# KikeM/romtime

Measured on AMD Instinct MI355X. Metric: snapshot-DoF/s for POD build, higher is better.
Workload: dtype f64

## Files before the change

### include/romtime_hip.h

```cpp
#ifndef ROMTIME_HIP_H
#define ROMTIME_HIP_H

#include <stdint.h>

#ifdef __cplusplus
extern "C" {
#endif

typedef struct rt_ctx rt_ctx;

#define RT_OK 0
#define RT_ERR_ARG (-1)
#define RT_ERR_HIP (-2)
#define RT_ERR_UNSUPPORTED (-3)
#define RT_WARN_ZERO_NORM 1
#define RT_WARN_SINGULAR 2

#define RT_ROW_MAJOR 0
#define RT_COL_MAJOR 1

int rt_version(void);
int rt_ctx_create(rt_ctx** out, int device);
void rt_ctx_destroy(rt_ctx* ctx);
int rt_ctx_set_stream(rt_ctx* ctx, void* hip_stream);
// ... 108 lines not shown
  const double* C_nl;
  const double* S_nl;
} rt_hsweep_desc;
int rt_hrom_bdf_sweep(rt_ctx* ctx, const rt_hsweep_desc* desc, double* uN_out);
int rt_last_sweep_stats(rt_ctx* ctx, int64_t* stats4);

int rt_trajectory_errors(rt_ctx* ctx, const double* B, int64_t ldb, const double* A, int64_t lda, int64_t stride_a,
                         const double* U, int64_t ldu, int u_layout, int64_t stride_u, int64_t N, int64_t k, int64_t nt,
                         int64_t n_traj, double* err, double* ref);

#define RT_P1_MASS 0
#define RT_P1_STIFFNESS 1
#define RT_P1_CONVECTION 2
#define RT_P1_TRILINEAR 3
#define RT_P1_LOAD 4
#define RT_P1_LOAD_P2 5
int rt_p1_local_assembly(rt_ctx* ctx, int kind, int64_t nx, const int64_t* rows, const int64_t* cols, int64_t m,
                         int64_t n_states, const double* h, const double* coef, int state_mode, const double* state,
                         double* out);

int rt_sym_eig_values(rt_ctx* ctx, const double* G, int64_t n, double* lam, int* status);
int rt_sym_eig_values_part(rt_ctx* ctx, const double* G, int64_t n, int64_t first, int64_t count, double* lam,
                           int* status);
int rt_sym_eig_vectors(rt_ctx* ctx, int64_t n, int64_t k, const double* lam, double* W);

int rt_host_jacobi_eigh(double* A, int64_t n, double* W, double* lam, int max_sweeps, int* sweeps_done);

int rt_bench_mfma_f64(rt_ctx* ctx, int iters, double* tflops);
int rt_bench_copy(rt_ctx* ctx, void* dst, const void* src, int64_t bytes, int reps, double* gbps);

#ifdef __cplusplus
}
#endif
#endif
```

### romtime_amd/_lib.py

```python
from __future__ import annotations

import ctypes as C
import os
import threading
import weakref

_HERE = os.path.dirname(os.path.abspath(__file__))
LIB_PATH = os.path.join(_HERE, "lib", "libromtime_hip.so")

ROW_MAJOR, COL_MAJOR = 0, 1
RT_OK = 0
WARN_ZERO_NORM, WARN_SINGULAR = 1, 2

_p = C.c_void_p
_i64 = C.c_int64
_int = C.c_int

SOLVER_DIRECT, SOLVER_GMRES = 0, 1


class GmresOpts(C.Structure):

    _fields_ = [("rtol", C.c_double), ("atol", C.c_double), ("restart", _i64), ("maxiter", _i64)]

# ... 21 lines not shown
    "rt_pod_enqueue": (_int, [_p, _p, _i64, _i64, _i64, _int, _i64, _int, _p, _p, _p, _p, _p, _p, _p]),
    "rt_pod_orth": (_int, [_p, _p, _i64, _i64, _i64, _int, _i64, C.c_double, _int, _p, _i64, C.POINTER(_i64), _p, _p,
                           C.POINTER(_int)]),
    "rt_gemm_tn": (_int, [_p, _p, _i64, _int, _p, _i64, _int, _i64, _i64, _i64, _p, _i64]),
    "rt_gemm_nn": (_int, [_p, _p, _i64, _int, _p, _i64, _i64, _i64, _i64, _p, _i64, _int]),
    "rt_rank_update": (_int, [_p, _p, _i64, _p, _p, _i64, _p, _i64, _i64, _i64, _i64, C.c_double, _p, _i64]),
    "rt_gemm_nn_axpby": (_int, [_p, _p, _i64, _int, _p, _i64, _i64, _i64, _i64, C.c_double, C.c_double, _p, _i64, _int]),
    "rt_transpose": (_int, [_p, _p, _i64, _i64, _i64, _p, _i64]),
    "rt_deim_greedy": (_int, [_p, _p, _i64, _i64, _i64, _int, _p, _p, _p]),
    "rt_csr_spmm": (_int, [_p, _p, _p, _p, _i64, _p, _i64, _i64, _p, _i64]),
    "rt_project_csr": (_int, [_p, _p, _p, _p, _i64, _p, _i64, _i64, _p]),
    "rt_project_csr_batched": (_int, [_p, _p, _p, _p, _i64, _int, _i64, _i64, _p, _i64, _i64, _p]),
    "rt_dense_solve_batched": (_int, [_p, _p, _p, _i64, _i64, _p]),
    "rt_dense_solve_multi": (_int, [_p, _p, _i64, _p, _p, _i64, _p]),
    "rt_tracked_solve_batched": (_int, [_p, _p, _p, _p, _i64, _i64, _int, _p]),
    "rt_gmres_batched": (_int, [_p, _p, _p, _p, _i64, _i64, C.POINTER(GmresOpts), _p, _p]),
    "rt_ctx_set_reduced_solver": (_int, [_p, _int, C.POINTER(GmresOpts)]),
    "rt_rom_bdf_sweep": (_int, [_p, _p, _p]),
    "rt_hrom_bdf_sweep": (_int, [_p, _p, _p]),
    "rt_trajectory_errors": (_int, [_p, _p, _i64, _p, _i64, _i64, _p, _i64, _int, _i64, _i64, _i64, _i64, _i64, _p, _p]),
    "rt_p1_local_assembly": (_int, [_p, _int, _i64, _p, _p, _i64, _i64, _p, _p, _int, _p, _p]),
    "rt_sym_eig_values": (_int, [_p, _p, _i64, _p, _p]),
    "rt_sym_eig_values_part": (_int, [_p, _p, _i64, _i64, _i64, _p, _p]),
    "rt_sym_eig_vectors": (_int, [_p, _i64, _i64, _p, _p]),
    "rt_host_jacobi_eigh": (_int, [_p, _i64, _p, _p, _int, C.POINTER(_int)]),
    "rt_bench_mfma_f64": (_int, [_p, _int, C.POINTER(C.c_double)]),
    "rt_bench_copy": (_int, [_p, _p, _p, _i64, _int, C.POINTER(C.c_double)]),
}



class SweepDesc(C.Structure):

    _fields_ = [("N", _i64), ("nnz", _i64), ("r", _i64), ("n_mu", _i64), ("nt", _i64), ("dt", C.c_double),
                ("bdf2", _int), ("indptr", _p), ("indices", _p), ("V", _p), ("mass_values", _p), ("n_terms", _i64),
                ("term_values", _p), ("term_coef", _p), ("tril_values", _p), ("n_rhs", _i64), ("rhs_terms", _p),
                ("rhs_coef", _p)]


class HSweepDesc(C.Structure):

    _fields_ = [("r", _i64), ("n_mu", _i64), ("nt", _i64), ("dt", C.c_double), ("bdf2", _int), ("m_mass", _i64),
                ("m_lin", _i64), ("m_nl", _i64), ("m_rhs", _i64), ("Z", _p), ("Zf", _p), ("F_mass", _p), ("F_lin", _p),
                ("F_rhs", _p), ("W", _p), ("C_nl", _p), ("S_nl", _p)]


# ... 165 lines not shown
```

### romtime_amd/csrc/api.hip

```cpp
#include "common.h"

#include <chrono>
#include <new>

typedef double d4 __attribute__((ext_vector_type(4)));

namespace {

int grow(rt_ctx* ctx, void** buf, size_t* have, size_t bytes, void** out) {
  if (bytes > *have) {
    RT_HIP_CHECK(ctx, hipStreamSynchronize(ctx->stream));
    if (*buf) RT_HIP_CHECK(ctx, hipFree(*buf));
    *buf = nullptr;
    *have = 0;
    const size_t want = (bytes + ((size_t)1 << 20) - 1) & ~(((size_t)1 << 20) - 1);
    RT_HIP_CHECK(ctx, hipMalloc(buf, want));
    *have = want;
  }
  *out = *buf;
  return RT_OK;
}

__global__ void gram_scale_kernel(double* __restrict__ G, int n, double* __restrict__ colnorm, int normalize,
                                  int* status_flag) {
// ... 111 lines not shown
__global__ __launch_bounds__(256) void copy_kernel(double4* __restrict__ dst, const double4* __restrict__ src, long n4) {
  const long stride = (long)gridDim.x * blockDim.x;
  for (long i = (long)blockIdx.x * blockDim.x + threadIdx.x; i < n4; i += stride) dst[i] = src[i];
}

}

int rt_scratch(rt_ctx* ctx, size_t bytes, void** out) { return grow(ctx, &ctx->scratch, &ctx->scratch_bytes, bytes, out); }
int rt_scratch2(rt_ctx* ctx, size_t bytes, void** out) {
  ++ctx->scratch2_gen;
  return grow(ctx, &ctx->scratch2, &ctx->scratch2_bytes, bytes, out);
}

int rt_func_lds(rt_ctx* ctx, const void* fn, int bytes) {
  for (const void* f : ctx->lds_done)
    if (f == fn) return RT_OK;
  RT_HIP_CHECK(ctx, hipFuncSetAttribute(fn, hipFuncAttributeMaxDynamicSharedMemorySize, bytes));
  ctx->lds_done.push_back(fn);
  return RT_OK;
}

extern "C" {

int rt_version(void) { return 340; }

int rt_ctx_create(rt_ctx** out, int device) {
  if (!out) return RT_ERR_ARG;
  *out = nullptr;
  int count = 0;
  if (hipGetDeviceCount(&count) != hipSuccess || device < 0 || device >= count) return RT_ERR_HIP;
  if (hipSetDevice(device) != hipSuccess) return RT_ERR_HIP;
  rt_ctx* ctx = new (std::nothrow) rt_ctx();
  if (!ctx) return RT_ERR_HIP;
  ctx->device = device;
  hipDeviceProp_t prop;
  if (hipGetDeviceProperties(&prop, device) == hipSuccess) ctx->num_cus = ctx->device_cus = prop.multiProcessorCount;
  if (hipMalloc(reinterpret_cast<void**>(&ctx->dev_counters), sizeof(long) * RT_N_COUNTERS) != hipSuccess ||
      hipMemset(ctx->dev_counters, 0, sizeof(long) * RT_N_COUNTERS) != hipSuccess) {
    delete ctx;
    return RT_ERR_HIP;
  }
  *out = ctx;
  return RT_OK;
}

void rt_ctx_destroy(rt_ctx* ctx) {
  if (!ctx) return;
// ... 44 lines not shown
int rt_ctx_synchronize(rt_ctx* ctx) {
  if (!ctx) return RT_ERR_ARG;
  RT_HIP_CHECK(ctx, hipStreamSynchronize(ctx->stream));
  return RT_OK;
}

const char* rt_last_error(rt_ctx* ctx) { return ctx ? ctx->err.c_str() : "null ctx"; }

int rt_last_launch_info(rt_ctx* ctx, int64_t* info3) {
  if (!ctx || !info3) return RT_ERR_ARG;
  info3[0] = ctx->last_grid;
  info3[1] = ctx->last_splits;
  info3[2] = ctx->last_tile;
  return RT_OK;
}

int rt_ctx_set_option(rt_ctx* ctx, const char* name, int value) {
  if (!ctx || !name) return RT_ERR_ARG;
  const std::string key(name);
  if (key == "eig_one_xcd") {
    ctx->eig_one_xcd = value != 0;
    return RT_OK;
  }
  if (key == "eig_xcd") {
    if (value < 0 || value > 7) {
      ctx->err = "rt_ctx_set_option: eig_xcd must be 0 .. 7";
      return RT_ERR_ARG;
    }
    ctx->eig_xcd = value;
    return RT_OK;
  }
  if (key == "gram_pace") {
    ctx->gram_pace_on = value != 0;
    return RT_OK;
  }
  if (key == "sweep_graph") {
    ctx->sweep_graph = value != 0;
    return RT_OK;
  }
  if (key == "cu_limit") {
    if (value < 0 || value > ctx->device_cus || (value % 8) != 0) {
      ctx->err = "rt_ctx_set_option: cu_limit must be a multiple of 8 between 0 and the device's CU count";
      return RT_ERR_ARG;
    }
    ctx->num_cus = value ? value : ctx->device_cus;
    return RT_OK;
  }
  ctx->err = "rt_ctx_set_option: unknown option " + key;
  return RT_ERR_ARG;
}

int rt_ctx_get_counter(rt_ctx* ctx, const char* name, int64_t* value) {
  if (!ctx || !name || !value) return RT_ERR_ARG;
  const std::string key(name);
  static const struct { const char* name; int slot; } table[] = {
      {"eig_timeouts", RT_CNT_EIG_TIMEOUT}, {"eig_general_form", RT_CNT_EIG_GENERAL_FORM},
      {"eig_one_xcd", RT_CNT_EIG_ONE_XCD}, {"gram_off_xcd", RT_CNT_GRAM_OFF_XCD}, {"sweep_newton_iterations", RT_CNT_NS_ITER},
      {"sweep_restarts", RT_CNT_NS_RESTART}, {"sweep_lu_fallbacks", RT_CNT_LU_FALLBACK}, {"sweep_solves", RT_CNT_SOLVES},
      {"sweep_gmres_iterations", RT_CNT_GMRES_ITER}, {"sweep_gmres_unconverged", RT_CNT_GMRES_UNCONVERGED}};
  for (const auto& t : table)
    if (key == t.name) {
      long host = 0;
      RT_HIP_CHECK(ctx, hipMemcpyAsync(&host, ctx->dev_counters + t.slot, sizeof(long), hipMemcpyDeviceToHost, ctx->stream));
      RT_HIP_CHECK(ctx, hipStreamSynchronize(ctx->stream));
      *value = host;
      return RT_OK;
    }
  ctx->err = "rt_ctx_get_counter: unknown counter " + key;
  return RT_ERR_ARG;
}

int rt_last_sweep_stats(rt_ctx* ctx, int64_t* stats4) {
  if (!ctx || !stats4) return RT_ERR_ARG;
  long host[4];
  RT_HIP_CHECK(ctx, hipMemcpyAsync(host, ctx->dev_counters + RT_CNT_NS_ITER, sizeof(host), hipMemcpyDeviceToHost, ctx->stream));
  RT_HIP_CHECK(ctx, hipStreamSynchronize(ctx->stream));
  for (int i = 0; i < 4; ++i) stats4[i] = host[i];
  return RT_OK;
}

int rt_ctx_set_profile(rt_ctx* ctx, int on) {
  if (!ctx) return RT_ERR_ARG;
// ... 175 lines not shown
```

### romtime_amd/csrc/common.h

```cpp
#pragma once
#include <hip/hip_runtime.h>
#include <stdint.h>
#include <string>
#include <vector>

#include "../../include/romtime_hip.h"

constexpr int RT_N_COUNTERS = 10;

struct rt_ctx {
  int device = 0;
  hipStream_t stream = nullptr;
  void* scratch = nullptr;
  size_t scratch_bytes = 0;
  void* scratch2 = nullptr;
  size_t scratch2_bytes = 0;
  int num_cus = 256;
  int device_cus = 256;
  std::string err;
  int64_t last_grid = 0, last_splits = 0, last_tile = 0;
  bool profile = false;
  hipEvent_t ev0 = nullptr, ev1 = nullptr;
  bool ev_valid = false;
  hipEvent_t gev0 = nullptr, gev1 = nullptr;
  bool gev_valid = false;
  bool sweep_graph = false;
  bool eig_one_xcd = true;
  int eig_xcd = 0;
  struct {
    const double *d = nullptr, *e = nullptr, *V = nullptr, *tau = nullptr;
    int64_t n = 0;
    void* base = nullptr;
    uint64_t gen = 0;
  } eig;
  uint64_t scratch2_gen = 0;
  std::vector<const void*> lds_done;
  long* dev_counters = nullptr;
  unsigned long long* gram_pace = nullptr;
  bool gram_pace_on = true;
  int reduced_solver = RT_SOLVER_DIRECT;
  rt_gmres_opts gmres_opts{1e-5, 0.0, 20, 1};
};

enum {
  RT_CNT_EIG_TIMEOUT = 0,
  RT_CNT_EIG_GENERAL_FORM = 1,
  RT_CNT_EIG_ONE_XCD = 2,
  RT_CNT_GRAM_OFF_XCD = 3,
  RT_CNT_NS_ITER = 4,
  RT_CNT_NS_RESTART = 5,
  RT_CNT_LU_FALLBACK = 6,
  RT_CNT_SOLVES = 7,
  RT_CNT_GMRES_ITER = 8,
  RT_CNT_GMRES_UNCONVERGED = 9
};

#define RT_TRY(expr)                 \
  do {                               \
    const int _rc = (expr);          \
    if (_rc != RT_OK) return _rc;    \
  } while (0)

int rt_func_lds(rt_ctx* ctx, const void* fn, int bytes);

#define RT_HIP_CHECK(ctx, expr)                                                              \
  do {                                                                                       \
    hipError_t _e = (expr);                                                                  \
    if (_e != hipSuccess) {                                                                  \
      (ctx)->err = std::string(#expr) + ": " + hipGetErrorString(_e);                        \
      return RT_ERR_HIP;                                                                     \
    }                                                                                        \
  } while (0)

#define RT_ARG_CHECK(ctx, cond)                                                              \
  do {                                                                                       \
    if (!(cond)) {                                                                           \
      (ctx)->err = std::string("bad argument: ") + #cond;                                    \
// ... 40 lines not shown
```

### romtime_amd/csrc/symeig.hip

```cpp
#include "common.h"
#include "wave_ops.h"

namespace {

constexpr int TW_SMALL = 32;
constexpr int SLOT0 = 160;
constexpr int TW_LARGE = 128;
constexpr int LPR = 64;
constexpr int TT = 1024;
static_assert(LPR == 64, "row reductions use the whole-wave DPP sum");
constexpr int NMAX = 1024;
constexpr int VEC_ITERS = 2;

struct TriParams {
  const double* G;
  double* V;
  double* P;
  double* tau;
  double* d;
  double* e;
  int* flags;
  int n;
  int tw;
  int local;
// ... 310 lines not shown
  double q = d[0] - x;
  if (fabs(q) < pivmin) q = -pivmin;
  int c = (q < 0.0);
  for (int i = 1; i < n; ++i) {
    q = fma(-e2[i - 1], fast_rcp(q), d[i] - x);
    if (fabs(q) < pivmin) q = -pivmin;
    c += (q < 0.0);
  }
  return c;
}

__global__ void symeig_init_kernel(int* flags, double* tau, int n) {
  for (int i = threadIdx.x; i < SLOT0 + TW_LARGE; i += blockDim.x) flags[i] = 0;
  for (int i = threadIdx.x; i < n; i += blockDim.x) tau[i] = 0.0;
}

constexpr int BIS_NS = 2;
template <int NM>
__global__ __launch_bounds__(256) void symeig_bisect_kernel(const double* __restrict__ d, const double* __restrict__ e,
                                                            int n, int first, int count, double* __restrict__ lam,
                                                            const int* flags, int* status, long* counters) {
  if (blockIdx.x == 0 && threadIdx.x == 0) {
    if (status) *status = flags[3];
    if (flags[3]) atomicAdd(reinterpret_cast<unsigned long long*>(&counters[RT_CNT_EIG_TIMEOUT]), 1ull);
  }
  __shared__ double sd[NM], se2[NM];
  __shared__ int s_first[2][4];
  const int tid = threadIdx.x, lane = tid & 63, wid = tid >> 6, half = wid & 1;
  double glo = 1e300, ghi = -1e300, emax = 0.0;
  for (int i = lane; i < n; i += 64) {
    const double di = d[i], ei = (i + 1 < n) ? e[i] : 0.0, el = (i > 0) ? fabs(e[i - 1]) : 0.0;
    sd[i] = di;
    se2[i] = ei * ei;
    glo = fmin(glo, di - el - fabs(ei));
    ghi = fmax(ghi, di + el + fabs(ei));
    emax = fmax(emax, ei * ei);
  }
  glo = rtw::wave_min(glo);
  ghi = rtw::wave_max(ghi);
  emax = rtw::wave_max(emax);
  __syncthreads();
  const double tn = fmax(fabs(glo), fabs(ghi));
  double lo = glo - 2.2e-16 * tn * n - 1e-300, hi = ghi + 2.2e-16 * tn * n + 1e-300;
  const double pivmin = 2.2250738585072014e-308 * fmax(1.0, emax);
  const int j = first + min(2 * (int)blockIdx.x + (wid >> 1), count - 1);
  const int want = n - j;
  constexpr int NSH = 128 * BIS_NS;
// ... 11 lines not shown
      q0 = fma(-ei, fast_rcp(q0), di - x0);
      q1 = fma(-ei, fast_rcp(q1), di - x1);
      if (fabs(q0) < pivmin) q0 = -pivmin;
      if (fabs(q1) < pivmin) q1 = -pivmin;
      c0 += (q0 < 0.0); c1 += (q1 < 0.0);
    }
    int first = NSH;
    if (c1 >= want) first = s0 + 1;
    if (c0 >= want) first = s0;
    first = rtw::wave_min_i32(first);
    if (lane == 0) s_first[pass & 1][wid] = first;
    __syncthreads();
    first = min(s_first[pass & 1][wid & 2], s_first[pass & 1][(wid & 2) + 1]);
    if (first == NSH) {
      lo = lo + h * NSH;
    } else {
      hi = lo + h * (first + 1);
      lo = lo + h * first;
    }
  }
  if (lane == 0 && half == 0) lam[j] = 0.5 * (lo + hi);
}

struct VecParams {
  const double* d;
  const double* e;
  const double* lam;
  const double* V;
  const double* tau;
  const double* C;
  double* W;
  int n, k;
};

constexpr int RBK = 4;

template <int NM>
__global__ __launch_bounds__(64) void symeig_wy_kernel(const double* __restrict__ V, int n, double* __restrict__ C) {
  constexpr int PER = NM / 64;
  const int b = blockIdx.x, lane = threadIdx.x, k0 = n - 3 - RBK * b;
  double v[RBK][PER];
#pragma unroll
  for (int u = 0; u < RBK; ++u)
#pragma unroll
    for (int q = 0; q < PER; ++q) {
      const int k = k0 - u, j = lane + 64 * q;
// ... 126 lines not shown
      a[u] = dot;
    }
#pragma unroll
    for (int u = 0; u < RBK; ++u) a[u] = rtw::wave_sum(a[u]);
    const double s0 = tk[0] * a[0];
    const double s1 = tk[1] * (a[1] - cc[0] * s0);
    const double s2 = tk[2] * (a[2] - cc[1] * s0 - cc[2] * s1);
    const double s3 = tk[3] * (a[3] - cc[3] * s0 - cc[4] * s1 - cc[5] * s2);
#pragma unroll
    for (int q = 0; q < PER; ++q)
      zr[q] = fma(-s3, vc[3][q], fma(-s2, vc[2][q], fma(-s1, vc[1][q], fma(-s0, vc[0][q], zr[q]))));
#pragma unroll
    for (int u = 0; u < RBK; ++u)
#pragma unroll
      for (int q = 0; q < PER; ++q) vc[u][q] = vn[u][q];
  }
#pragma unroll
  for (int q = 0; q < PER; ++q) {
    const int j = lane + 64 * q;
    if (j < n) z[j] = zr[q];
  }
  __syncthreads();
  for (int i = lane; i < n; i += 64) p.W[(size_t)i * p.k + t] = z[i];
}

}

extern "C" int rt_sym_eig_values(rt_ctx* ctx, const double* G, int64_t n, double* lam, int* status) {
  return rt_sym_eig_values_part(ctx, G, n, 0, n, lam, status);
}

extern "C" int rt_sym_eig_values_part(rt_ctx* ctx, const double* G, int64_t n, int64_t first, int64_t count, double* lam,
                                      int* status) {
  if (!ctx) return RT_ERR_ARG;
  RT_ARG_CHECK(ctx, G && lam && n >= 3 && first >= 0 && count >= 1 && first + count <= n);
  if (n > NMAX) {
    ctx->err = "rt_sym_eig_values: n > 1024 not supported (the matrix must stay resident in the LDS of <= 128 CUs)";
    return RT_ERR_UNSUPPORTED;
  }
  const bool large = n > 512;
  const bool small_team = !large && ctx->num_cus < TW_SMALL && ctx->num_cus >= TW_SMALL / 2;
  int tw = large ? TW_LARGE : (small_team ? TW_SMALL / 2 : TW_SMALL);
  const bool local = n <= 64;
  if (local) tw = 1;
  if (tw > ctx->num_cus) {
    ctx->err = "rt_sym_eig_values: not enough compute units for the cooperative tridiagonalisation";
// ... 21 lines not shown

  const int RB = (int)((n + tw - 1) / tw);
  const size_t lds = sizeof(double) * ((size_t)RB * (local ? n + 2 : n) + 5 * n + 16);
  const bool tiny = n <= 256, tinier = n <= 128;
  RT_TRY(rt_func_lds(ctx, reinterpret_cast<const void*>(&symeig_tridiag_kernel<128>), 150 * 1024));
  RT_TRY(rt_func_lds(ctx, reinterpret_cast<const void*>(&symeig_tridiag_kernel<256>), 150 * 1024));
  RT_TRY(rt_func_lds(ctx, reinterpret_cast<const void*>(&symeig_tridiag_kernel<512>), 150 * 1024));
  RT_TRY(rt_func_lds(ctx, reinterpret_cast<const void*>(&symeig_tridiag_kernel<1024>), 150 * 1024));
  {
    int per_cu = 0;
    if (large)
      RT_HIP_CHECK(ctx, hipOccupancyMaxActiveBlocksPerMultiprocessor(&per_cu, symeig_tridiag_kernel<1024>, TT, lds));
    else if (tinier)
      RT_HIP_CHECK(ctx, hipOccupancyMaxActiveBlocksPerMultiprocessor(&per_cu, symeig_tridiag_kernel<128>, TT, lds));
    else if (tiny)
      RT_HIP_CHECK(ctx, hipOccupancyMaxActiveBlocksPerMultiprocessor(&per_cu, symeig_tridiag_kernel<256>, TT, lds));
    else
      RT_HIP_CHECK(ctx, hipOccupancyMaxActiveBlocksPerMultiprocessor(&per_cu, symeig_tridiag_kernel<512>, TT, lds));
    if ((long)per_cu * ctx->num_cus < tw) {
      ctx->err = "rt_sym_eig_values: the device cannot keep all cooperating workgroups resident";
      return RT_ERR_UNSUPPORTED;
    }
  }
  const dim3 bgrid((unsigned)((count + 1) / 2));
  if (large) {
    hipLaunchKernelGGL(symeig_tridiag_kernel<1024>, dim3(tw), dim3(TT), lds, st, tp);
    RT_HIP_CHECK(ctx, hipGetLastError());
    hipLaunchKernelGGL(symeig_bisect_kernel<1024>, bgrid, dim3(256), 0, st, tp.d, tp.e, (int)n, (int)first, (int)count,
                       lam, tp.flags, status, ctx->dev_counters);
  } else {
    if (tinier)
      hipLaunchKernelGGL(symeig_tridiag_kernel<128>, dim3(tp.spread ? 16 * tw : tw), dim3(TT), lds, st, tp);
    else if (tiny)
      hipLaunchKernelGGL(symeig_tridiag_kernel<256>, dim3(tp.spread ? 16 * tw : tw), dim3(TT), lds, st, tp);
    else
      hipLaunchKernelGGL(symeig_tridiag_kernel<512>, dim3(tp.spread ? 16 * tw : tw), dim3(TT), lds, st, tp);
    RT_HIP_CHECK(ctx, hipGetLastError());
    hipLaunchKernelGGL(symeig_bisect_kernel<512>, bgrid, dim3(256), 0, st, tp.d, tp.e, (int)n, (int)first, (int)count,
                       lam, tp.flags, status, ctx->dev_counters);
  }
  RT_HIP_CHECK(ctx, hipGetLastError());
  ctx->eig.d = tp.d; ctx->eig.e = tp.e; ctx->eig.V = tp.V; ctx->eig.tau = tp.tau; ctx->eig.n = n; ctx->eig.base = base;
  ctx->eig.gen = ctx->scratch2_gen;
  return RT_OK;
}

extern "C" int rt_sym_eig_vectors(rt_ctx* ctx, int64_t n, int64_t k, const double* lam, double* W) {
  if (!ctx) return RT_ERR_ARG;
  RT_ARG_CHECK(ctx, lam && W && k >= 1 && k <= n);
  if (ctx->eig.n != n || ctx->eig.base == nullptr || ctx->eig.base != ctx->scratch2 || ctx->eig.gen != ctx->scratch2_gen) {
    ctx->err = "rt_sym_eig_vectors: must follow rt_sym_eig_values on the same ctx and matrix with no other composite "
               "operator (greedy, projection, sweep) in between";
    return RT_ERR_ARG;
  }
  VecParams vp;
  vp.d = ctx->eig.d; vp.e = ctx->eig.e; vp.lam = lam; vp.V = ctx->eig.V; vp.tau = ctx->eig.tau;
  vp.W = W; vp.n = (int)n; vp.k = (int)k;
  const int nblk = (int)((n - 2 + RBK - 1) / RBK);
  void* cbuf = nullptr;
  int rc = rt_scratch(ctx, sizeof(double) * 6 * (size_t)nblk, &cbuf);
  if (rc != RT_OK) return rc;
  vp.C = static_cast<const double*>(cbuf);
  RT_TRY(rt_func_lds(ctx, reinterpret_cast<const void*>(&symeig_vectors_kernel<128>), 80 * 1024));
  RT_TRY(rt_func_lds(ctx, reinterpret_cast<const void*>(&symeig_vectors_kernel<256>), 80 * 1024));
  RT_TRY(rt_func_lds(ctx, reinterpret_cast<const void*>(&symeig_vectors_kernel<512>), 80 * 1024));
  RT_TRY(rt_func_lds(ctx, reinterpret_cast<const void*>(&symeig_vectors_kernel<1024>), 80 * 1024));
  if (n > 512) {
// ... 24 lines not shown
```

### romtime_amd/csrc/wave_ops.h

```cpp
#pragma once
#include <hip/hip_runtime.h>

namespace rtw {

template <int CTRL, int ROW_MASK = 0xf, int BANK_MASK = 0xf>
__device__ __forceinline__ double dpp_f64(double x) {
  const long long b = __double_as_longlong(x);
  int lo = (int)b, hi = (int)(b >> 32);
  lo = __builtin_amdgcn_update_dpp(0, lo, CTRL, ROW_MASK, BANK_MASK, false);
  hi = __builtin_amdgcn_update_dpp(0, hi, CTRL, ROW_MASK, BANK_MASK, false);
  return __longlong_as_double(((long long)hi << 32) | (unsigned)lo);
}

__device__ __forceinline__ double read_lane(double x, int lane) {
  const long long b = __double_as_longlong(x);
  const int lo = __builtin_amdgcn_readlane((int)b, lane), hi = __builtin_amdgcn_readlane((int)(b >> 32), lane);
  return __longlong_as_double(((long long)hi << 32) | (unsigned)lo);
}

__device__ __forceinline__ double first_lane(double x) {
  const long long b = __double_as_longlong(x);
  const int lo = __builtin_amdgcn_readfirstlane((int)b), hi = __builtin_amdgcn_readfirstlane((int)(b >> 32));
  return __longlong_as_double(((long long)hi << 32) | (unsigned)lo);
}
// ... 29 lines not shown
  return read_lane(x, 63);
}

__device__ __forceinline__ double wave_min(double x) {
  x = fmin(x, dpp_keep_f64<0xb1>(x));
  x = fmin(x, dpp_keep_f64<0x4e>(x));
  x = fmin(x, dpp_keep_f64<0x114>(x));
  x = fmin(x, dpp_keep_f64<0x118>(x));
  x = fmin(x, dpp_keep_f64<0x142, 0xa>(x));
  x = fmin(x, dpp_keep_f64<0x143, 0xc>(x));
  return read_lane(x, 63);
}

__device__ __forceinline__ int wave_min_i32(int x) {
  x = min(x, dpp_keep_i32<0xb1>(x));
  x = min(x, dpp_keep_i32<0x4e>(x));
  x = min(x, dpp_keep_i32<0x114>(x));
  x = min(x, dpp_keep_i32<0x118>(x));
  x = min(x, dpp_keep_i32<0x142, 0xa>(x));
  x = min(x, dpp_keep_i32<0x143, 0xc>(x));
  return __builtin_amdgcn_readlane(x, 63);
}

template <int CTRL, int ROW_MASK = 0xf, int BANK_MASK = 0xf>
__device__ __forceinline__ void argmax_step(double& v, int& i) {
  const double ov = dpp_keep_f64<CTRL, ROW_MASK, BANK_MASK>(v);
  const int oi = dpp_keep_i32<CTRL, ROW_MASK, BANK_MASK>(i);
  const bool take = ov > v || (ov == v && oi < i);
  v = take ? ov : v;
  i = take ? oi : i;
}
__device__ __forceinline__ void wave_argmax(double& v, int& i) {
  argmax_step<0xb1>(v, i);
  argmax_step<0x4e>(v, i);
  argmax_step<0x114>(v, i);
  argmax_step<0x118>(v, i);
  argmax_step<0x142, 0xa>(v, i);
  argmax_step<0x143, 0xc>(v, i);
  v = read_lane(v, 63);
  i = __builtin_amdgcn_readlane(i, 63);
}

}
```

### romtime_amd/ops.py

```python
from __future__ import annotations

import ctypes as C

import numpy as np
import torch

from . import _lib
from ._lib import COL_MAJOR, ROW_MAJOR, Context, RomtimeHipError

_p = C.c_void_p


def _ptr(t):
    return _p(t.data_ptr()) if t is not None else _p(None)


def _need_gpu():
    if not torch.cuda.is_available():
        raise RomtimeHipError("no MI355X visible: romtime_amd's hot path runs on the GPU only (there is no CPU fallback)")


def to_device(a, device=None) -> torch.Tensor:
    _need_gpu()
    if isinstance(a, torch.Tensor):
# ... 324 lines not shown
    elif poly is not None:
        st = to_device(poly).contiguous()
        if tuple(st.shape) != (n_states, 3):
            raise RomtimeHipError("p1_local_assembly: `poly` must be (n_states, 3)")
        mode = 3
    out = torch.empty((n_states, m), dtype=torch.float64, device=h.device)
    ctx.check(ctx.lib.rt_p1_local_assembly(ctx.handle, P1_KINDS[kind], int(nx), _ptr(rows), _ptr(cols), m, n_states, _ptr(h),
                                           _ptr(coef), mode, _ptr(st), _ptr(out)), "rt_p1_local_assembly")
    return out


def sym_eig_values(G: torch.Tensor, first: int = 0, count: int | None = None):
    ctx = Context.current()
    n = G.shape[0]
    assert G.is_contiguous() and G.shape == (n, n)
    count = n - first if count is None else count
    lam = torch.empty(n, dtype=torch.float64, device=G.device)
    status = torch.zeros(1, dtype=torch.int32, device=G.device)
    ctx.check(ctx.lib.rt_sym_eig_values_part(ctx.handle, _ptr(G), n, first, count, _ptr(lam), _ptr(status)),
              "rt_sym_eig_values_part")
    return lam, status


def sym_eig_vectors(lam: torch.Tensor, k: int, first: int = 0) -> torch.Tensor:
    ctx = Context.current()
    n = lam.numel()
    W = torch.empty((n, k), dtype=torch.float64, device=lam.device)
    ctx.check(ctx.lib.rt_sym_eig_vectors(ctx.handle, n, k, _ptr(lam[first:]), _ptr(W)), "rt_sym_eig_vectors")
    return W


def transpose(src: torch.Tensor) -> torch.Tensor:
    ctx = Context.current()
    src = src.contiguous()
    rows, cols = src.shape
    dst = torch.empty((cols, rows), dtype=torch.float64, device=src.device)
    ctx.check(ctx.lib.rt_transpose(ctx.handle, _ptr(src), rows, cols, cols, _ptr(dst), rows), "rt_transpose")
    return dst


def bench_mfma_f64(iters: int = 20000) -> float:
    ctx = Context.current()
    out = C.c_double()
    ctx.check(ctx.lib.rt_bench_mfma_f64(ctx.handle, iters, C.byref(out)), "rt_bench_mfma_f64")
    return out.value

# ... 9 lines not shown
```

### romtime_amd/pipeline.py

```python
from __future__ import annotations

import collections
import ctypes as C
import os
import weakref

import numpy as np
import torch

from . import _lib, ops, pod

_p = C.c_void_p


SMALL_SET = 150_000_000
_STREAMS: dict = {}
_STREAMS_PID: list = []
_OPEN_RUNS = weakref.WeakSet()


def shutdown():
    import gc

    if not _STREAMS:
# ... 92 lines not shown

                    dist.all_reduce(Gbuf, op=dist.ReduceOp.SUM, group=self.group)
                item["g"] = torch.cuda.Event(enable_timing=True)
                item["g"].record()
        if self.sR is not None:
            import torch.distributed as dist

            with torch.cuda.stream(self.sR):
                self.sR.wait_event(item["k0"])
                dist.all_reduce(Gbuf, op=dist.ReduceOp.SUM, group=self.group)
                item["g"] = torch.cuda.Event(enable_timing=True)
                item["g"].record()

    def _eig(self, item):
        k, normalize = item["k"], item["normalize"]
        item["owner"] = item["index"] % self.world
        if self.rank != item["owner"]:
            return
        with self.ctxE.use(self.sE):
            self.sE.wait_event(item["g"])
            G = item["G"]
            n = G.shape[0]
            colnorm, flag = ops.gram_scale(G, normalize)
            lam_d, status = ops.sym_eig_values(G)
            Z = ops.sym_eig_vectors(lam_d, k)
            Zs = ops.backproject_weights(Z, lam_d, colnorm if normalize else None)
            item["payload"] = torch.cat([lam_d, colnorm, status.to(torch.float64), flag.to(torch.float64), Zs.reshape(-1)])
            item["_keep"] = (lam_d, status, flag, Z, Zs, colnorm)
            item["ec"] = torch.cuda.Event(enable_timing=True)
            item["ec"].record()

    def _share(self, item):
        n, k = item["G"].shape[0], item["k"]
        st = self.sE if self.group_e is None else self.sC
        with torch.cuda.stream(st):
            if self.group_e is not None:
                import torch.distributed as dist

                if self.rank == item["owner"]:
                    st.wait_event(item["ec"])
                else:
                    item["payload"] = torch.empty(n * (k + 2) + 2, dtype=torch.float64, device=item["G"].device)
                dist.broadcast(item["payload"], src=dist.get_global_rank(self.group_e, item["owner"]), group=self.group_e)
            payload = item["payload"]
            item["colnorm"].copy_(payload[n:2 * n])
            item["Zs"] = payload[2 * n + 2:].view(n, k)
            head = torch.cat([payload[:n], payload[2 * n:2 * n + 2], item["Gbuf"][-1:]])
            item["head"] = torch.empty(head.numel(), dtype=torch.float64).pin_memory()
            item["head"].copy_(head, non_blocking=True)
            item["_keep2"] = head
            item["e"] = torch.cuda.Event(enable_timing=True)
            item["e"].record()

    def _backproject(self, item):
        ctx, st = self.ctxG, self.sG
        with ctx.use(st):
            st.wait_event(item["e"])
            ops.gemm_nn(item["X"], item["Zs"], out=item["Q"])
            item["b"] = torch.cuda.Event(enable_timing=True)
            item["b"].record()

    def _regular(self, item):
        self.recomputed += 1
        self.sE.synchronize()
        return pod.pod_device(item["X"], num=item["num"], normalize=item["normalize"], group=self.group)

    def _finish(self, item):
        if item["direct"]:
            return self._regular(item)
        item["b"].synchronize()
        n, k = item["X"].shape[1], item["k"]
        head = item["head"].numpy()
        lam, status, zero_norm, n_rows = head[:n], int(head[n]), int(head[n + 1]), int(round(head[n + 2]))
        if item["normalize"] and zero_norm:
            raise ValueError("array must not contain infs or NaNs (zero-norm snapshot with normalize=True)")
        s = np.sqrt(np.clip(lam, 0.0, None))
        energy = pod._energy(s)
        gaps = lam[:k] - lam[1:k + 1] if k < n else np.r_[lam[:k - 1] - lam[1:k], lam[k - 1]]
        ok = (status == 0 and s[0] > 0 and s[k - 1] >= pod.TWO_PASS_RATIO * s[0]
              and gaps.min() >= pod.RR_GAP * max(lam[0], 1e-300) and n_rows >= n)
        self.last_stage_ms = dict(gram_kernel_ms=item["t0"].elapsed_time(item["k0"]),
                                  gram_allreduce_ms=item["t0"].elapsed_time(item["g"]),
                                  eig_chain_ms=item["g"].elapsed_time(item["e"]),
                                  gram_start_to_basis_ms=item["t0"].elapsed_time(item["b"]))
        self.gram_kernel_ms.append(self.last_stage_ms["gram_kernel_ms"])
        if not ok:
            return self._regular(item)
        return dict(Q=item["Q"], s=s, energy=energy, VT=None, r=k, passes=1, colnorm=item["colnorm"])

    def run(self, snapshot_sets, num, normalize=True, depth=2):
        if not num:
            raise ValueError("PodPipeline enqueues ahead of the spectrum: it needs `num` (pod.py:51-53)")
        gen = self._run(snapshot_sets, num, normalize, depth)
        _OPEN_RUNS.add(gen)
        return gen

    def _run(self, snapshot_sets, num, normalize, depth):
        main = torch.cuda.current_stream(self.device)
        flight = collections.deque()
        it = iter(snapshot_sets)
        self._admitted = 0
        depth = max(depth, self.world + 1)

        def after_producer():
            ready = torch.cuda.Event()
            ready.record(main)
            for st in (self.sG, self.sE, self.sC):
                if st is not None:
                    st.wait_event(ready)

        materialised = isinstance(snapshot_sets, (list, tuple))
        if materialised:
            after_producer()

        def admit():
            try:
                X = next(it)
            except StopIteration:
                return None
            if X.dim() != 2 or not X.is_cuda or X.dtype != torch.float64:
                raise _lib.RomtimeHipError("PodPipeline takes 2-D float64 CUDA tensors")
            item = dict(X=X, num=num, k=int(min(num, X.shape[1])), normalize=bool(normalize), index=self._admitted)
            self._admitted += 1
            n = X.shape[1]
            rows = X.shape[0] * self.world
            item["direct"] = not (3 <= n <= 512) or rows * n < self.small_set
            if not item["direct"]:
                item["Q"] = torch.empty((X.shape[0], item["k"]), dtype=torch.float64, device=X.device)
                item["colnorm"] = torch.empty(n, dtype=torch.float64, device=X.device)
                if not materialised:
                    after_producer()
                self._gram(item)
                self._eig(item)
            return item

        pending = collections.deque()
        for _ in range(self.world):
            item = admit()
            if item is None:
                break
            pending.append(item)
        while pending:
            cur = pending.popleft()
            if not cur["direct"]:
                self._share(cur)
            nxt = admit()
            if nxt is not None:
                pending.append(nxt)
            if not cur["direct"]:
                self._backproject(cur)
            flight.append(cur)
            while len(flight) > depth or (not pending and flight):
                yield self._finish(flight.popleft())
        done = torch.cuda.Event()
        done.record(self.sG)
        main.wait_event(done)
        done2 = torch.cuda.Event()
        done2.record(self.sE)
        main.wait_event(done2)
        if self.sC is not None:
            done3 = torch.cuda.Event()
            done3.record(self.sC)
            main.wait_event(done3)

    def map(self, snapshot_sets, num, normalize=True, depth=2):
        return list(self.run(snapshot_sets, num, normalize=normalize, depth=depth))


class PodLanes:

    def __init__(self, lanes: int = 8, device=None):
        if not torch.cuda.is_available():
            raise _lib.RomtimeHipError("no MI355X visible: romtime_amd's hot path runs on the GPU only")
        if not (1 <= int(lanes) <= 8):
            raise ValueError("lanes must be 1 .. 8 (one per XCD)")
        self.device = torch.device("cuda", torch.cuda.current_device() if device is None else device)
        self.ctx, self.streams = [], []
        for lane in range(int(lanes)):
            c = _lib.Context(self.device.index)
            c.set_option("eig_xcd", lane)
            self.ctx.append(c)
            self.streams.append(torch.cuda.Stream(self.device))
        self.recomputed = 0

    def close(self):
        torch.cuda.synchronize(self.device)

    def _enqueue(self, item, lane):
        X, k, normalize = item["X"], item["k"], item["normalize"]
# ... 173 lines not shown
```

Before: 88.58 billion.

## Split eigenvalue bisection into leading-k and deferred rest with lean multisection kernel

The symmetric eigenvalue stage now computes only the leading k eigenvalues first, then builds the weights and signals the backprojection GEMM. The remaining eigenvalues are computed afterwards on the same stream so they overlap with the basis GEMM. Eigenvalues past 2*num_cus use a new lean multisection bisection kernel that packs several eigenvalues per wavefront, with DPP group-min reductions. In the single-process case the pipeline also admits more items ahead (lead) and runs the share step inline. This adds scheduling complexity, and finish now waits on the full eig event.

```diff
diff --git a/include/romtime_hip.h b/include/romtime_hip.h
--- a/include/romtime_hip.h
+++ b/include/romtime_hip.h
@@ -154,6 +154,7 @@
 int rt_sym_eig_values(rt_ctx* ctx, const double* G, int64_t n, double* lam, int* status);
 int rt_sym_eig_values_part(rt_ctx* ctx, const double* G, int64_t n, int64_t first, int64_t count, double* lam,
                            int* status);
+int rt_sym_eig_values_rest(rt_ctx* ctx, int64_t n, int64_t first, int64_t count, double* lam, int* status);
 int rt_sym_eig_vectors(rt_ctx* ctx, int64_t n, int64_t k, const double* lam, double* W);
 
 int rt_host_jacobi_eigh(double* A, int64_t n, double* W, double* lam, int max_sweeps, int* sweeps_done);
diff --git a/romtime_amd/_lib.py b/romtime_amd/_lib.py
--- a/romtime_amd/_lib.py
+++ b/romtime_amd/_lib.py
@@ -67,6 +67,7 @@
     "rt_p1_local_assembly": (_int, [_p, _int, _i64, _p, _p, _i64, _i64, _p, _p, _int, _p, _p]),
     "rt_sym_eig_values": (_int, [_p, _p, _i64, _p, _p]),
     "rt_sym_eig_values_part": (_int, [_p, _p, _i64, _i64, _i64, _p, _p]),
+    "rt_sym_eig_values_rest": (_int, [_p, _i64, _i64, _i64, _p, _p]),
     "rt_sym_eig_vectors": (_int, [_p, _i64, _i64, _p, _p]),
     "rt_host_jacobi_eigh": (_int, [_p, _i64, _p, _p, _int, C.POINTER(_int)]),
     "rt_bench_mfma_f64": (_int, [_p, _int, C.POINTER(C.c_double)]),
diff --git a/romtime_amd/csrc/api.hip b/romtime_amd/csrc/api.hip
--- a/romtime_amd/csrc/api.hip
+++ b/romtime_amd/csrc/api.hip
@@ -157,7 +157,7 @@
 
 extern "C" {
 
-int rt_version(void) { return 340; }
+int rt_version(void) { return 350; }
 
 int rt_ctx_create(rt_ctx** out, int device) {
   if (!out) return RT_ERR_ARG;
@@ -248,6 +248,10 @@
     ctx->eig_one_xcd = value != 0;
     return RT_OK;
   }
+  if (key == "eig_lean") {
+    ctx->eig_lean = value != 0;
+    return RT_OK;
+  }
   if (key == "eig_xcd") {
     if (value < 0 || value > 7) {
       ctx->err = "rt_ctx_set_option: eig_xcd must be 0 .. 7";
@@ -283,7 +287,8 @@
       {"eig_timeouts", RT_CNT_EIG_TIMEOUT}, {"eig_general_form", RT_CNT_EIG_GENERAL_FORM},
       {"eig_one_xcd", RT_CNT_EIG_ONE_XCD}, {"gram_off_xcd", RT_CNT_GRAM_OFF_XCD}, {"sweep_newton_iterations", RT_CNT_NS_ITER},
       {"sweep_restarts", RT_CNT_NS_RESTART}, {"sweep_lu_fallbacks", RT_CNT_LU_FALLBACK}, {"sweep_solves", RT_CNT_SOLVES},
-      {"sweep_gmres_iterations", RT_CNT_GMRES_ITER}, {"sweep_gmres_unconverged", RT_CNT_GMRES_UNCONVERGED}};
+      {"sweep_gmres_iterations", RT_CNT_GMRES_ITER}, {"sweep_gmres_unconverged", RT_CNT_GMRES_UNCONVERGED},
+      {"eig_lean_multisections", RT_CNT_EIG_LEAN}};
   for (const auto& t : table)
     if (key == t.name) {
       long host = 0;
diff --git a/romtime_amd/csrc/common.h b/romtime_amd/csrc/common.h
--- a/romtime_amd/csrc/common.h
+++ b/romtime_amd/csrc/common.h
@@ -6,7 +6,7 @@
 
 #include "../../include/romtime_hip.h"
 
-constexpr int RT_N_COUNTERS = 10;
+constexpr int RT_N_COUNTERS = 11;
 
 struct rt_ctx {
   int device = 0;
@@ -26,9 +26,11 @@
   bool gev_valid = false;
   bool sweep_graph = false;
   bool eig_one_xcd = true;
+  bool eig_lean = true;
   int eig_xcd = 0;
   struct {
     const double *d = nullptr, *e = nullptr, *V = nullptr, *tau = nullptr;
+    const int* flags = nullptr;
     int64_t n = 0;
     void* base = nullptr;
     uint64_t gen = 0;
@@ -52,7 +54,8 @@
   RT_CNT_LU_FALLBACK = 6,
   RT_CNT_SOLVES = 7,
   RT_CNT_GMRES_ITER = 8,
-  RT_CNT_GMRES_UNCONVERGED = 9
+  RT_CNT_GMRES_UNCONVERGED = 9,
+  RT_CNT_EIG_LEAN = 10
 };
 
 #define RT_TRY(expr)                 \
diff --git a/romtime_amd/csrc/symeig.hip b/romtime_amd/csrc/symeig.hip
--- a/romtime_amd/csrc/symeig.hip
+++ b/romtime_amd/csrc/symeig.hip
@@ -1,3 +1,5 @@
+#include <algorithm>
+
 #include "common.h"
 #include "wave_ops.h"
 
@@ -356,7 +358,7 @@
                                                             const int* flags, int* status, long* counters) {
   if (blockIdx.x == 0 && threadIdx.x == 0) {
     if (status) *status = flags[3];
-    if (flags[3]) atomicAdd(reinterpret_cast<unsigned long long*>(&counters[RT_CNT_EIG_TIMEOUT]), 1ull);
+    if (flags[3] && counters) atomicAdd(reinterpret_cast<unsigned long long*>(&counters[RT_CNT_EIG_TIMEOUT]), 1ull);
   }
   __shared__ double sd[NM], se2[NM];
   __shared__ int s_first[2][4];
@@ -414,6 +416,81 @@
   if (lane == 0 && half == 0) lam[j] = 0.5 * (lo + hi);
 }
 
+#ifndef ROMTIME_LEAN_LPE
+#define ROMTIME_LEAN_LPE 16
+#endif
+constexpr int LEAN_LPE = ROMTIME_LEAN_LPE;
+template <int NM, int LPE>
+__global__ __launch_bounds__(256) void symeig_bisect_lean_kernel(const double* __restrict__ d, const double* __restrict__ e,
+                                                                 int n, int first, int count, double* __restrict__ lam,
+                                                                 const int* flags, int* status, long* counters,
+                                                                 int count_timeout) {
+  static_assert(LPE == 16 || LPE == 32, "two rounds per pass: LPE shifts, then 256 / LPE - 1");
+  if (blockIdx.x == 0 && threadIdx.x == 0) {
+    if (status) *status = flags[3];
+    if (flags[3] && count_timeout) atomicAdd(reinterpret_cast<unsigned long long*>(&counters[RT_CNT_EIG_TIMEOUT]), 1ull);
+    atomicAdd(reinterpret_cast<unsigned long long*>(&counters[RT_CNT_EIG_LEAN]), 1ull);
+  }
+  __shared__ double sd[NM], se2[NM];
+  const int tid = threadIdx.x, lane = tid & 63, wid = tid >> 6;
+  double glo = 1e300, ghi = -1e300, emax = 0.0;
+  for (int i = lane; i < n; i += 64) {
+    const double di = d[i], ei = (i + 1 < n) ? e[i] : 0.0, el = (i > 0) ? fabs(e[i - 1]) : 0.0;
+    sd[i] = di;
+    se2[i] = ei * ei;
+    glo = fmin(glo, di - el - fabs(ei));
+    ghi = fmax(ghi, di + el + fabs(ei));
+    emax = fmax(emax, ei * ei);
+  }
+  glo = rtw::wave_min(glo);
+  ghi = rtw::wave_max(ghi);
+  emax = rtw::wave_max(emax);
+  __syncthreads();
+  const double tn = fmax(fabs(glo), fabs(ghi));
+  double lo = glo - 2.2e-16 * tn * n - 1e-300, hi = ghi + 2.2e-16 * tn * n + 1e-300;
+  const double pivmin = 2.2250738585072014e-308 * fmax(1.0, emax);
+  constexpr int EPW = 64 / LPE;
+  constexpr int NSH = 128 * BIS_NS;
+  constexpr int NSEC = NSH + 1;
+  constexpr int BLK = NSH / LPE;
+  const int sub = lane % LPE;
+  const int idx = EPW * (4 * (int)blockIdx.x + wid) + lane / LPE;
+  const int j = first + min(idx, count - 1);
+  const int want = n - j;
+  auto reaches = [&](double h, int s) {
+    const int s0 = s & ~1;
+    const double x0 = lo + h * (s0 + 1);
+    const double x = (s & 1) ? x0 + h : x0;
+    double q = sd[0] - x;
+    if (fabs(q) < pivmin) q = -pivmin;
+    int c = (q < 0.0);
+    for (int i = 1; i < n; ++i) {
+      q = fma(-se2[i - 1], fast_rcp(q), sd[i] - x);
+      if (fabs(q) < pivmin) q = -pivmin;
+      c += (q < 0.0);
+    }
+    return c >= want;
+  };
+  for (int pass = 0; pass < 7; ++pass) {
+    const double h = (hi - lo) / NSEC;
+    int blk = reaches(h, BLK * sub + BLK - 1) ? sub : LPE;
+    blk = rtw::group_min_i32<LPE>(blk);
+    int first = NSH;
+    if (blk < LPE) {
+      const int s = BLK * blk + min(sub, BLK - 2);
+      first = (sub < BLK - 1 && reaches(h, s)) ? s : BLK * blk + BLK - 1;
+    }
+    first = rtw::group_min_i32<LPE>(first);
+    if (first == NSH) {
+      lo = lo + h * NSH;
+    } else {
+      hi = lo + h * (first + 1);
+      lo = lo + h * first;
+    }
+  }
+  if (sub == 0 && idx < count) lam[j] = 0.5 * (lo + hi);
+}
+
 struct VecParams {
   const double* d;
   const double* e;
@@ -586,6 +663,40 @@
   }
   __syncthreads();
   for (int i = lane; i < n; i += 64) p.W[(size_t)i * p.k + t] = z[i];
+}
+
+int launch_multisection(rt_ctx* ctx, const double* d, const double* e, const int* flags, int64_t n, int64_t first,
+                        int64_t count, double* lam, int* status, bool first_instalment) {
+  hipStream_t st = ctx->stream;
+  const int64_t end = first + count;
+  const int64_t lean_from = ctx->eig_lean ? 2 * (int64_t)ctx->num_cus : n;
+  const int64_t n_lat = std::min(end, lean_from) - first;
+  const int64_t lean_first = std::max(first, lean_from);
+  bool count_timeout = first_instalment;
+  if (n_lat > 0) {
+    const dim3 grid((unsigned)((n_lat + 1) / 2));
+    long* counters = count_timeout ? ctx->dev_counters : nullptr;
+    if (n > 512)
+      hipLaunchKernelGGL(symeig_bisect_kernel<1024>, grid, dim3(256), 0, st, d, e, (int)n, (int)first, (int)n_lat, lam,
+                         flags, status, counters);
+    else
+      hipLaunchKernelGGL(symeig_bisect_kernel<512>, grid, dim3(256), 0, st, d, e, (int)n, (int)first, (int)n_lat, lam,
+                         flags, status, counters);
+    RT_HIP_CHECK(ctx, hipGetLastError());
+    count_timeout = false;
+  }
+  if (lean_first < end) {
+    const int64_t n_lean = end - lean_first;
+    const dim3 grid((unsigned)((n_lean + 4 * (64 / LEAN_LPE) - 1) / (4 * (64 / LEAN_LPE))));
+    if (n > 512)
+      hipLaunchKernelGGL((symeig_bisect_lean_kernel<1024, LEAN_LPE>), grid, dim3(256), 0, st, d, e, (int)n,
+                         (int)lean_first, (int)n_lean, lam, flags, status, ctx->dev_counters, count_timeout ? 1 : 0);
+    else
+      hipLaunchKernelGGL((symeig_bisect_lean_kernel<512, LEAN_LPE>), grid, dim3(256), 0, st, d, e, (int)n,
+                         (int)lean_first, (int)n_lean, lam, flags, status, ctx->dev_counters, count_timeout ? 1 : 0);
+    RT_HIP_CHECK(ctx, hipGetLastError());
+  }
+  return RT_OK;
 }
 
 }
@@ -653,12 +764,8 @@
       return RT_ERR_UNSUPPORTED;
     }
   }
-  const dim3 bgrid((unsigned)((count + 1) / 2));
   if (large) {
     hipLaunchKernelGGL(symeig_tridiag_kernel<1024>, dim3(tw), dim3(TT), lds, st, tp);
-    RT_HIP_CHECK(ctx, hipGetLastError());
-    hipLaunchKernelGGL(symeig_bisect_kernel<1024>, bgrid, dim3(256), 0, st, tp.d, tp.e, (int)n, (int)first, (int)count,
-                       lam, tp.flags, status, ctx->dev_counters);
   } else {
     if (tinier)
       hipLaunchKernelGGL(symeig_tridiag_kernel<128>, dim3(tp.spread ? 16 * tw : tw), dim3(TT), lds, st, tp);
@@ -666,14 +773,24 @@
       hipLaunchKernelGGL(symeig_tridiag_kernel<256>, dim3(tp.spread ? 16 * tw : tw), dim3(TT), lds, st, tp);
     else
       hipLaunchKernelGGL(symeig_tridiag_kernel<512>, dim3(tp.spread ? 16 * tw : tw), dim3(TT), lds, st, tp);
-    RT_HIP_CHECK(ctx, hipGetLastError());
-    hipLaunchKernelGGL(symeig_bisect_kernel<512>, bgrid, dim3(256), 0, st, tp.d, tp.e, (int)n, (int)first, (int)count,
-                       lam, tp.flags, status, ctx->dev_counters);
   }
   RT_HIP_CHECK(ctx, hipGetLastError());
+  RT_TRY(launch_multisection(ctx, tp.d, tp.e, tp.flags, n, first, count, lam, status, true));
   ctx->eig.d = tp.d; ctx->eig.e = tp.e; ctx->eig.V = tp.V; ctx->eig.tau = tp.tau; ctx->eig.n = n; ctx->eig.base = base;
+  ctx->eig.flags = tp.flags;
   ctx->eig.gen = ctx->scratch2_gen;
   return RT_OK;
+}
+
+extern "C" int rt_sym_eig_values_rest(rt_ctx* ctx, int64_t n, int64_t first, int64_t count, double* lam, int* status) {
+  if (!ctx) return RT_ERR_ARG;
+  RT_ARG_CHECK(ctx, lam && n >= 3 && first >= 0 && count >= 1 && first + count <= n);
+  if (ctx->eig.n != n || ctx->eig.base == nullptr || ctx->eig.base != ctx->scratch2 || ctx->eig.gen != ctx->scratch2_gen) {
+    ctx->err = "rt_sym_eig_values_rest: must follow rt_sym_eig_values_part on the same ctx and matrix with no other "
+               "composite operator (greedy, projection, sweep) in between";
+    return RT_ERR_ARG;
+  }
+  return launch_multisection(ctx, ctx->eig.d, ctx->eig.e, ctx->eig.flags, n, first, count, lam, status, false);
 }
 
 extern "C" int rt_sym_eig_vectors(rt_ctx* ctx, int64_t n, int64_t k, const double* lam, double* W) {
diff --git a/romtime_amd/csrc/wave_ops.h b/romtime_amd/csrc/wave_ops.h
--- a/romtime_amd/csrc/wave_ops.h
+++ b/romtime_amd/csrc/wave_ops.h
@@ -75,6 +75,25 @@
   return __builtin_amdgcn_readlane(x, 63);
 }
 
+template <int G>
+__device__ __forceinline__ int group_min_i32(int x) {
+  static_assert(G == 16 || G == 32, "a DPP row or half a wave");
+  x = min(x, dpp_keep_i32<0xb1>(x));
+  x = min(x, dpp_keep_i32<0x4e>(x));
+  x = min(x, dpp_keep_i32<0x114>(x));
+  x = min(x, dpp_keep_i32<0x118>(x));
+  const int g = (threadIdx.x & 63) / G;
+  if constexpr (G == 32) {
+    x = min(x, dpp_keep_i32<0x142, 0xa>(x));
+    const int a = __builtin_amdgcn_readlane(x, 31), b = __builtin_amdgcn_readlane(x, 63);
+    return g ? b : a;
+  } else {
+    const int a = __builtin_amdgcn_readlane(x, 15), b = __builtin_amdgcn_readlane(x, 31), c = __builtin_amdgcn_readlane(x, 47),
+              d = __builtin_amdgcn_readlane(x, 63);
+    return g == 0 ? a : g == 1 ? b : g == 2 ? c : d;
+  }
+}
+
 template <int CTRL, int ROW_MASK = 0xf, int BANK_MASK = 0xf>
 __device__ __forceinline__ void argmax_step(double& v, int& i) {
   const double ov = dpp_keep_f64<CTRL, ROW_MASK, BANK_MASK>(v);
diff --git a/romtime_amd/ops.py b/romtime_amd/ops.py
--- a/romtime_amd/ops.py
+++ b/romtime_amd/ops.py
@@ -370,6 +370,15 @@
     return lam, status
 
 
+def sym_eig_values_rest(lam: torch.Tensor, first: int, count: int | None = None, status: torch.Tensor | None = None):
+    ctx = Context.current()
+    n = lam.numel()
+    assert lam.is_contiguous() and lam.dtype == torch.float64
+    count = n - first if count is None else count
+    ctx.check(ctx.lib.rt_sym_eig_values_rest(ctx.handle, n, first, count, _ptr(lam), _ptr(status)), "rt_sym_eig_values_rest")
+    return lam
+
+
 def sym_eig_vectors(lam: torch.Tensor, k: int, first: int = 0) -> torch.Tensor:
     ctx = Context.current()
     n = lam.numel()
diff --git a/romtime_amd/pipeline.py b/romtime_amd/pipeline.py
--- a/romtime_amd/pipeline.py
+++ b/romtime_amd/pipeline.py
@@ -138,13 +138,25 @@
             G = item["G"]
             n = G.shape[0]
             colnorm, flag = ops.gram_scale(G, normalize)
-            lam_d, status = ops.sym_eig_values(G)
-            Z = ops.sym_eig_vectors(lam_d, k)
-            Zs = ops.backproject_weights(Z, lam_d, colnorm if normalize else None)
+            if self.group_e is None:
+                lam_d, status = ops.sym_eig_values(G, 0, k)
+                Z = ops.sym_eig_vectors(lam_d, k)
+                Zs = ops.backproject_weights(Z, lam_d, colnorm if normalize else None)
+                item["Zs"] = Zs
+                item["z"] = torch.cuda.Event(enable_timing=True)
+                item["z"].record()
+                if k < n:
+                    ops.sym_eig_values_rest(lam_d, k)
+            else:
+                lam_d, status = ops.sym_eig_values(G)
+                Z = ops.sym_eig_vectors(lam_d, k)
+                Zs = ops.backproject_weights(Z, lam_d, colnorm if normalize else None)
             item["payload"] = torch.cat([lam_d, colnorm, status.to(torch.float64), flag.to(torch.float64), Zs.reshape(-1)])
             item["_keep"] = (lam_d, status, flag, Z, Zs, colnorm)
             item["ec"] = torch.cuda.Event(enable_timing=True)
             item["ec"].record()
+        if self.group_e is None:
+            self._share(item)
 
     def _share(self, item):
         n, k = item["G"].shape[0], item["k"]
@@ -160,7 +172,8 @@
                 dist.broadcast(item["payload"], src=dist.get_global_rank(self.group_e, item["owner"]), group=self.group_e)
             payload = item["payload"]
             item["colnorm"].copy_(payload[n:2 * n])
-            item["Zs"] = payload[2 * n + 2:].view(n, k)
+            if self.group_e is not None:
+                item["Zs"] = payload[2 * n + 2:].view(n, k)
             head = torch.cat([payload[:n], payload[2 * n:2 * n + 2], item["Gbuf"][-1:]])
             item["head"] = torch.empty(head.numel(), dtype=torch.float64).pin_memory()
             item["head"].copy_(head, non_blocking=True)
@@ -171,7 +184,7 @@
     def _backproject(self, item):
         ctx, st = self.ctxG, self.sG
         with ctx.use(st):
-            st.wait_event(item["e"])
+            st.wait_event(item["z"] if self.group_e is None else item["e"])
             ops.gemm_nn(item["X"], item["Zs"], out=item["Q"])
             item["b"] = torch.cuda.Event(enable_timing=True)
             item["b"].record()
@@ -185,6 +198,7 @@
         if item["direct"]:
             return self._regular(item)
         item["b"].synchronize()
+        item["e"].synchronize()
         n, k = item["X"].shape[1], item["k"]
         head = item["head"].numpy()
         lam, status, zero_norm, n_rows = head[:n], int(head[n]), int(head[n + 1]), int(round(head[n + 2]))
@@ -199,24 +213,29 @@
                                   gram_allreduce_ms=item["t0"].elapsed_time(item["g"]),
                                   eig_chain_ms=item["g"].elapsed_time(item["e"]),
                                   gram_start_to_basis_ms=item["t0"].elapsed_time(item["b"]))
+        if "z" in item:
+            self.last_stage_ms["gram_end_to_weights_ms"] = item["k0"].elapsed_time(item["z"])
         self.gram_kernel_ms.append(self.last_stage_ms["gram_kernel_ms"])
         if not ok:
             return self._regular(item)
         return dict(Q=item["Q"], s=s, energy=energy, VT=None, r=k, passes=1, colnorm=item["colnorm"])
 
-    def run(self, snapshot_sets, num, normalize=True, depth=2):
+    def run(self, snapshot_sets, num, normalize=True, depth=2, lead=None):
         if not num:
             raise ValueError("PodPipeline enqueues ahead of the spectrum: it needs `num` (pod.py:51-53)")
-        gen = self._run(snapshot_sets, num, normalize, depth)
+        lead = max(2, self.world) if lead is None else int(lead)
+        if lead < 1:
+            raise ValueError("lead must be at least 1")
+        gen = self._run(snapshot_sets, num, normalize, depth, max(lead, self.world))
         _OPEN_RUNS.add(gen)
         return gen
 
-    def _run(self, snapshot_sets, num, normalize, depth):
+    def _run(self, snapshot_sets, num, normalize, depth, lead):
         main = torch.cuda.current_stream(self.device)
         flight = collections.deque()
         it = iter(snapshot_sets)
         self._admitted = 0
-        depth = max(depth, self.world + 1)
+        depth = max(depth, lead + 1)
 
         def after_producer():
             ready = torch.cuda.Event()
@@ -251,14 +270,14 @@
             return item
 
         pending = collections.deque()
-        for _ in range(self.world):
+        for _ in range(lead):
             item = admit()
             if item is None:
                 break
             pending.append(item)
         while pending:
             cur = pending.popleft()
-            if not cur["direct"]:
+            if not cur["direct"] and self.group_e is not None:
                 self._share(cur)
             nxt = admit()
             if nxt is not None:
@@ -279,8 +298,8 @@
             done3.record(self.sC)
             main.wait_event(done3)
 
-    def map(self, snapshot_sets, num, normalize=True, depth=2):
-        return list(self.run(snapshot_sets, num, normalize=normalize, depth=depth))
+    def map(self, snapshot_sets, num, normalize=True, depth=2, lead=None):
+        return list(self.run(snapshot_sets, num, normalize=normalize, depth=depth, lead=lead))
 
 
 class PodLanes:
```

After: 89.08 billion, median of 6. About the same (+0.6%).
